# Wikinaut/agrep

Measured on NVIDIA H100. Metric: text_scan_throughput, higher is better.
Workload: dtype u32 bitwise

## Files before the change

### agrep_b200/csrc/refine.cu

```cuda
#include "scan_internal.cuh"


#define REFINE_MAXG  8
int refine_launch_u32a(int nrows, const RefineParams &P, unsigned &grid, cudaStream_t st);
int refine_launch_u32b(int nrows, const RefineParams &P, unsigned &grid, cudaStream_t st);
int refine_launch_u64(int nrows, const RefineParams &P, unsigned &grid, cudaStream_t st);
int refine_launch_costs(bool narrow, int nrows, const RefineParams &P, unsigned &grid, cudaStream_t st);

__global__ void __launch_bounds__(REFINE_THREADS)
k_compact_ranges(const uint32_t *bitmap, uint64_t n_words, const uint64_t *range_offsets, uint64_t *list, uint64_t cap)
{
	const uint32_t lane = threadIdx.x & 31;
	const uint64_t warp = ((uint64_t)blockIdx.x * REFINE_THREADS + threadIdx.x) >> 5, nwarps = ((uint64_t)gridDim.x * REFINE_THREADS) >> 5;
	const uint64_t n_groups = (n_words + 31) / 32, per = (n_groups + nwarps - 1) / nwarps;
	const uint64_t g_begin = warp * per < n_groups ? warp * per : n_groups, g_end = (g_begin + per < n_groups) ? g_begin + per : n_groups;
	uint64_t at = range_offsets[warp];
	for (uint64_t g0 = g_begin; g0 < g_end; g0 += 8) {
		uint32_t wd[8];
#pragma unroll
		for (int u = 0; u < 8; u++) { const uint64_t w = (g0 + u) * 32 + lane; wd[u] = (g0 + u < g_end && w < n_words) ? bitmap[w] : 0u; }
#pragma unroll
		for (int u = 0; u < 8; u++) {
			const uint32_t word = wd[u];
			if (!__ballot_sync(0xffffffffu, word != 0)) continue;
			const uint64_t w = (g0 + u) * 32 + lane;
			uint32_t c = __popc(word), pre = c;
#pragma unroll
			for (int o = 1; o < 32; o <<= 1) { uint32_t v = __shfl_up_sync(0xffffffffu, pre, o); if (lane >= (uint32_t)o) pre += v; }
			const uint32_t total = __shfl_sync(0xffffffffu, pre, 31);
			uint64_t mine = at + (pre - c);
			for (uint32_t b = word; b; b &= b - 1) { if (mine < cap) list[mine] = w * 32 + (uint64_t)(__ffs(b) - 1); mine++; }
			at += total;
		}
	}
}

static bool refine_geometry(const agb_desc &d, RefineParams &P)
{
	if (!front_usable(d) || !d.refine) return false;
	int max_off = 0, min_off = 1 << 30;
	for (int i = 0; i < d.n_anchors; i++) { max_off = std::max(max_off, (int)d.anchor_off[i]); min_off = std::min(min_off, (int)d.anchor_off[i]); }
	for (int i = 0; i < d.n_anchors3; i++) { max_off = std::max(max_off, (int)d.anchor3_off[i]); min_off = std::min(min_off, (int)d.anchor3_off[i]); }
	P.lo_off = max_off + d.k;
	P.hi_off = 15 + d.pat_len - min_off + d.k;
	P.gb = (P.lo_off + 15) / 16;
	P.ng = P.gb + (P.hi_off + 15) / 16;
	if (P.ng < P.gb + 2) P.ng = P.gb + 2;
	const int pw = (d.pat_len + 3) / 4, ngc = (d.engine != AGB_ENGINE_ASEARCH1 && d.M <= 31 && pw <= 4) ? 4 : REFINE_MAXG;
	if (!(P.ng <= ngc && max_off <= 31 && d.pat_len >= 1 && d.pat_len <= 64)) return false;
	const int na = d.n_anchors + d.n_anchors3;
	if (na > 16) return false;
	uint32_t val[16], msk[16]; int off[16];
	for (int i = 0; i < d.n_anchors; i++) { val[i] = d.anchor[i]; msk[i] = d.anchor_mask; off[i] = d.anchor_off[i]; }
	for (int i = 0; i < d.n_anchors3; i++) { val[d.n_anchors + i] = d.anchor3[i]; msk[d.n_anchors + i] = 0x00FFFFFFu; off[d.n_anchors + i] = d.anchor3_off[i]; }
	for (int i = 0; i < na; i++) for (int j = 0; j < i; j++) if ((val[i] & msk[j]) == val[j] || (val[j] & msk[i]) == val[i]) return false;
	uint32_t mul = 0x9E3779B1u;
	for (int attempt = 0; attempt < 4096; attempt++, mul = mul * 0x2C1B3C6Du + 0x297A2D39u) {
		int8_t slot[32]; bool ok = true;
		memset(slot, 0, sizeof slot);
		mul |= 1u;
		for (int i = 0; i < na && ok; i++) {
			const uint32_t h = (val[i] * mul) >> 27;
			if (slot[h]) ok = false; else slot[h] = (int8_t)(i + 1);
		}
		if (!ok) continue;
		P.hmul = mul;
		memcpy(P.hidx64, slot, sizeof slot);
		int8_t offs8[16];
		for (int i = 0; i < 16; i++) { P.hval[i] = i < na ? val[i] : 0; P.hmask[i] = i < na ? msk[i] : 0; offs8[i] = i < na ? (int8_t)off[i] : 0; }
		memcpy(P.hoffs64, offs8, sizeof offs8);
		return true;
	}
	return false;
}

static void refine_t1_setup(const agb_desc &d, RefineParams &P)
{
	uint8_t lit[64]; bool is_lit[64]; bool fold = false; int n_lit = 0;
	for (int j = 0; j < d.pat_len; j++) {
		const uint64_t bit = 1ull << (d.M - (d.L + 2 + j));
		int cnt = 0, c0 = -1, c1 = -1;
		for (int c = 0; c < 256; c++) if (d.mask[c] & bit) { if (cnt == 0) c0 = c; else if (cnt == 1) c1 = c; cnt++; }
		is_lit[j] = false; lit[j] = 0;
		if (cnt == 1 && c0 < 0x80) { is_lit[j] = true; lit[j] = (uint8_t)c0; }
		else if (cnt == 2 && (c0 ^ c1) == 0x20 && c1 < 0x80) { is_lit[j] = true; lit[j] = (uint8_t)(c0 | 0x20); fold = true; }
		if (is_lit[j]) n_lit++;
	}
	P.t1 = 0;
	if (n_lit <= d.k + 1) return;
	P.t1 = 1; P.t1_fold = fold ? 0x20202020u : 0u;
	for (int w = 0; w < 16; w++) { P.t1_pat[w] = 0; P.t1_care[w] = 0; }
	for (int j = 0; j < d.pat_len; j++) if (is_lit[j]) {
		P.t1_pat[j >> 2] |= (uint32_t)(fold ? (lit[j] | 0x20) : lit[j]) << (8 * (j & 3));
		P.t1_care[j >> 2] |= 0x80u << (8 * (j & 3));
	}
}

int refine_launch(const agb_desc &d, Workspace &W, const void *d_text, uint64_t n, cudaStream_t st, bool *ran)
{
	RefineParams P; memset(&P, 0, sizeof P);
	*ran = false;
	if (n == 0 || !refine_geometry(d, P)) return AGB_OK;
	const uint64_t n_chunks = (n + 15) / 16, n_words = (n_chunks + 31) / 32;
	P.text = (const uint8_t *)d_text; P.bitmap = W.bitmap; P.out = W.bitmap2; P.warp_counts = W.range_counts;
	P.n = n; P.n_chunks = n_chunks; P.n_words = n_words; P.desc = W.d_desc;
	P.fold = d.anchor_fold; P.amask = d.anchor_mask; P.na = d.n_anchors; P.k = d.k; P.pat_len = d.pat_len;
	for (int i = 0; i < d.n_anchors; i++) { P.anchor[i] = d.anchor[i]; P.off[i] = d.anchor_off[i]; }
	{
		bool distinct = true;
		for (int i = 0; i < d.n_anchors; i++) for (int j = 0; j < i; j++) if (d.anchor[i] == d.anchor[j]) distinct = false;
		P.one = 1; P.scale = 1;
		for (int i = d.anchor_len; i < 4; i++) P.scale <<= 8;
		P.poly = (distinct && poly_setup(d.anchor, d.n_anchors, 8 * d.anchor_len, P.coef)) ? 1 : 0;
		P.n3 = 0;
		if (d.n_anchors3) {
			uint32_t c3[AGB_MAXANCHOR];
			if (!P.poly || !poly_setup(d.anchor3, d.n_anchors3, 24, c3)) return AGB_OK;
			P.n3 = d.n_anchors3;
			for (int i = 0; i < d.n_anchors3; i++) P.coef3[i] = c3[i];
		}
	}
	refine_t1_setup(d, P);
	unsigned grid = refine_grid(W, n);
	P.sm_count = W.sm_count;
	const bool costs = d.engine == AGB_ENGINE_ASEARCH1, narrow = d.M <= 31;
	int rc = costs ? refine_launch_costs(narrow, d.nrows, P, grid, st)
	       : !narrow ? refine_launch_u64(d.nrows, P, grid, st)
	       : d.nrows <= 4 ? refine_launch_u32a(d.nrows, P, grid, st) : refine_launch_u32b(d.nrows, P, grid, st);
	if (rc) return AGB_ERR_ARG;
	g_launches++;
	CUDA_TRY(cudaGetLastError());
	W.refine_ctas = grid;
	*ran = true;
	return AGB_OK;
}

unsigned refine_grid(const Workspace &W, uint64_t n)
{
	const uint64_t n_chunks = (n + 15) / 16, n_words = (n_chunks + 31) / 32, groups = (n_words + 31) / 32;
	unsigned grid = (unsigned)std::min<uint64_t>((groups + 3) / 4, (uint64_t)W.sm_count * 16);
	return grid ? grid : 1;
}

int compact_ranges_launch(Workspace &W, uint64_t n, cudaStream_t st)
{
	const uint64_t n_chunks = (n + 15) / 16, n_words = (n_chunks + 31) / 32;
	const unsigned grid = W.refine_ctas;
	k_compact_ranges<<<grid, REFINE_THREADS, 0, st>>>(W.bitmap2, n_words, W.range_offsets, W.cand, W.cand_cap); g_launches++;
	CUDA_TRY(cudaGetLastError());
	return AGB_OK;
}
```

### agrep_b200/csrc/refine_kernel.cuh

```cuda
#ifndef AGB_REFINE_KERNEL_CUH
#define AGB_REFINE_KERNEL_CUH
#include "automaton.cuh"

#define REFINE_RING1 544
#define REFINE_RING2 64
#define REFINE_RING3 128
#define REFINE_MAXG  8
#define REFINE_PAD   32

struct AnchorTable { int8_t idx[32]; uint32_t val[16], mask[16]; int8_t off[16]; int n; };
__device__ __forceinline__ uint32_t hit_windows_tab(const uint32_t (&x)[5], const AnchorTable &A)
{
	uint32_t hits = 0;
#pragma unroll
	for (int w = 0; w < 4; w++) {
		const uint32_t wv[4] = { x[w], __funnelshift_r(x[w], x[w + 1], 8), __funnelshift_r(x[w], x[w + 1], 16), __funnelshift_r(x[w], x[w + 1], 24) };
		for (int a = 0; a < A.n; a++) {
			const uint32_t V = A.val[a], M = A.mask[a];
#pragma unroll
			for (int j = 0; j < 4; j++) if ((wv[j] & M) == V) hits |= 1u << (4 * w + j);
		}
	}
	return hits;
}

template <int NA, bool SCALED>
__device__ __forceinline__ uint32_t hit_windows_poly(const uint32_t (&x)[5], const RefineParams &P)
{
	uint32_t wv[16];
#pragma unroll
	for (int w = 0; w < 4; w++) {
		wv[4 * w] = x[w]; wv[4 * w + 1] = __funnelshift_r(x[w], x[w + 1], 8);
		wv[4 * w + 2] = __funnelshift_r(x[w], x[w + 1], 16); wv[4 * w + 3] = __funnelshift_r(x[w], x[w + 1], 24);
	}
	uint32_t nz = 0;
#pragma unroll
	for (int s = 15; s >= 0; s--) {
		uint32_t r = wv[s] * P.one + P.coef[NA - 1];
#pragma unroll
		for (int i = NA - 2; i >= 0; i--) r = r * wv[s] + P.coef[i];
		if (SCALED) r *= P.scale;
		nz = nz * 2u + min(r, 1u);
	}
	return ~nz & 0xFFFFu;
}
__device__ __forceinline__ uint32_t hit_windows_cmp(const uint32_t (&x)[5], const RefineParams &P)
{
	uint32_t hits = 0;
#pragma unroll
	for (int w = 0; w < 4; w++) {
		const uint32_t wv[4] = { x[w], __funnelshift_r(x[w], x[w + 1], 8), __funnelshift_r(x[w], x[w + 1], 16), __funnelshift_r(x[w], x[w + 1], 24) };
		for (int a = 0; a < P.na; a++) {
			const uint32_t A = P.anchor[a];
#pragma unroll
			for (int j = 0; j < 4; j++) if ((wv[j] & P.amask) == A) hits |= 1u << (4 * w + j);
		}
	}
	return hits;
}
template <bool SCALED>
__device__ __forceinline__ uint32_t hit_windows_na(const uint32_t (&x)[5], const RefineParams &P)
{
	switch (P.na) {
	case 1: return hit_windows_poly<1, SCALED>(x, P);  case 2: return hit_windows_poly<2, SCALED>(x, P);
	case 3: return hit_windows_poly<3, SCALED>(x, P);  case 4: return hit_windows_poly<4, SCALED>(x, P);
	case 5: return hit_windows_poly<5, SCALED>(x, P);  case 6: return hit_windows_poly<6, SCALED>(x, P);
	case 7: return hit_windows_poly<7, SCALED>(x, P);  case 8: return hit_windows_poly<8, SCALED>(x, P);
	default: return hit_windows_poly<9, SCALED>(x, P);
	}
}
__device__ __forceinline__ uint32_t hit_windows(const uint32_t (&x)[5], const RefineParams &P)
{
	if (!P.poly) return hit_windows_cmp(x, P);
	return P.scale != 1 ? hit_windows_na<true>(x, P) : hit_windows_na<false>(x, P);
}

__device__ __forceinline__ uint32_t start_code(const uint32_t *cw, const int s, const RefineParams &P, const AnchorTable &A)
{
	const uint32_t lo = cw[s >> 2] | P.fold, hi = cw[(s >> 2) + 1] | P.fold;
	const uint32_t v = __funnelshift_r(lo, hi, (s & 3) * 8);
	int off = 0;
	{
		const uint32_t v4 = v & P.amask;
		const int i = A.idx[(v4 * P.hmul) >> 27];
		if (i && A.val[i - 1] == (v & A.mask[i - 1])) off = A.off[i - 1];
		else if (P.n3) {
			const uint32_t v3 = v & 0x00FFFFFFu;
			const int i3 = A.idx[(v3 * P.hmul) >> 27];
			if (i3 && A.val[i3 - 1] == (v & A.mask[i3 - 1])) off = A.off[i3 - 1];
		}
	}
	return (uint32_t)(32 + s - off);
}

template <int NW, int NWT, int ND>
__device__ __forceinline__ bool band_count_passes(const RefineParams &P, const uint32_t *strip, const int so)
{
	uint32_t W[NWT + 1];
	{
		const uint32_t *src = strip + (so >> 2);
		const uint32_t sh = ((uint32_t)so & 3u) * 8u;
		uint32_t Lw[NWT + 1];
#pragma unroll
		for (int i = 0; i <= NWT; i++) Lw[i] = src[i];
#pragma unroll
		for (int i = 0; i < NWT; i++) W[i] = (__funnelshift_r(Lw[i], Lw[i + 1], sh) & 0x7F7F7F7Fu) | P.t1_fold;
		W[NWT] = 0;
	}
	uint32_t acc[NW];
#pragma unroll
	for (int w = 0; w < NW; w++) acc[w] = 0x80808080u;
	const int nd = ND ? ND : 2 * P.k + 1;
#pragma unroll (ND ? ND : 1)
	for (int d = 0; d < nd; d++) {
#pragma unroll
		for (int w = 0; w < NW; w++) acc[w] &= (W[w] ^ P.t1_pat[w]) + 0x7F7F7F7Fu;
#pragma unroll
		for (int i = 0; i < NWT; i++) W[i] = __funnelshift_r(W[i], W[i + 1], 8);
	}
	int miss = 0;
#pragma unroll
	for (int w = 0; w < NW; w++) miss += __popc(acc[w] & P.t1_care[w]);
	return miss <= P.k;
}

template <typename T, int NR, bool COSTS>
__device__ __forceinline__ bool window_passes(const uint8_t *bytes, const bool run, const int wlen, const T init0,
                                              const T *mask, const DevConsts<T> &C)
{
	T S[NR];
#pragma unroll
	for (int r = 0; r < NR; r++) S[r] = init0;
	int q = 0;
	for (; q + 4 <= wlen; q += 4) {
		int c[4];
#pragma unroll
		for (int i = 0; i < 4; i++) c[i] = run ? (int)__ldg(bytes + q + i) : 0;
		T m[4];
#pragma unroll
		for (int i = 0; i < 4; i++) m[i] = mask[c[i]];
#pragma unroll
		for (int i = 0; i < 4; i++) rows_step<T, NR, COSTS>(S, m[i], C);
	}
	for (; q < wlen; q++) {
		const int c = run ? (int)__ldg(bytes + q) : 0;
		rows_step<T, NR, COSTS>(S, mask[c], C);
	}
	return run && (S[NR - 1] & C.endpos) != 0;
}

struct Refill { uint32_t word, next_word; uint32_t half; };
__device__ __forceinline__ void refine_refill(const RefineParams &P, Refill &R, uint32_t *ring, uint32_t &count, uint32_t lane,
                                              uint64_t &g, uint64_t g_begin, uint64_t g_end)
{
	if (R.half == 0) {
		const uint64_t w = g * 32 + lane;
		R.word = R.next_word;
		if (w < P.n_words) P.out[w] = 0u;
		R.next_word = (g + 1 < g_end && w + 32 < P.n_words) ? P.bitmap[w + 32] : 0u;
	}
	const uint32_t word = ((lane >> 4) == R.half) ? R.word : 0u;
	uint32_t c = __popc(word), pre = c;
#pragma unroll
	for (int o = 1; o < 32; o <<= 1) { uint32_t v = __shfl_up_sync(0xffffffffu, pre, o); if (lane >= (uint32_t)o) pre += v; }
	const uint32_t total = __shfl_sync(0xffffffffu, pre, 31);
	pre += count - c;
	const uint32_t rel0 = (uint32_t)(g - g_begin) * 1024u + lane * 32u;
	for (uint32_t b = word; b; b &= b - 1) ring[pre++] = rel0 + (uint32_t)(__ffs(b) - 1);
	count += total;
	if (R.half) g++;
	R.half ^= 1u;
	__syncwarp();
}

template <typename T, int NR, bool COSTS, int NW>
__global__ void __launch_bounds__(REFINE_THREADS, 6)
k_refine(const RefineParams P)
{
	constexpr int NGC = NW <= 4 ? 4 : REFINE_MAXG;
	constexpr int NWT = NW + (2 * (NR - 1) + 3) / 4;
	extern __shared__ __align__(16) uint32_t s_strip[];
	__shared__ RecShared<T, NR> SH;
	__shared__ uint32_t s_ring1[REFINE_THREADS / 32][REFINE_RING1];
	__shared__ uint32_t s_ring2[REFINE_THREADS / 32][REFINE_RING2];
	__shared__ uint32_t s_ring3[REFINE_THREADS / 32][REFINE_RING3];
	__shared__ AnchorTable s_offs;
	if (threadIdx.x == 0) {
#pragma unroll
		for (int i = 0; i < 32; i++) s_offs.idx[i] = (int8_t)(P.hidx64[i >> 3] >> (8 * (i & 7)));
#pragma unroll
		s_offs.n = P.na + P.n3;
#pragma unroll
		for (int i = 0; i < 16; i++) { s_offs.val[i] = P.hval[i]; s_offs.mask[i] = P.hmask[i]; s_offs.off[i] = (int8_t)(P.hoffs64[i >> 3] >> (8 * (i & 7))); }
	}
	DevConsts<T> C;
	shared_init<T, NR>(SH, C, P.desc, REFINE_THREADS);
	const T init0 = mirror<T>((T)P.desc->init0);
	const int wlen = P.pat_len + 2 * P.k;
	const uint32_t lane = threadIdx.x & 31, wib = threadIdx.x >> 5, lt_mask = (1u << lane) - 1u;
	uint32_t *ring1 = s_ring1[wib], *ring2 = s_ring2[wib], *ring3 = s_ring3[wib];
	const int stride_w = P.ng * 4 + 1;
	uint32_t *strip = s_strip + threadIdx.x * stride_w;
	const uint32_t *cw = strip + P.gb * 4;
	const int so0 = P.gb * 16 - 32 - P.k;

	const uint64_t warp = ((uint64_t)blockIdx.x * REFINE_THREADS + threadIdx.x) >> 5, nwarps = ((uint64_t)gridDim.x * REFINE_THREADS) >> 5;
	const uint64_t n_groups = (P.n_words + 31) / 32, per = (n_groups + nwarps - 1) / nwarps;
	const uint64_t g_begin = warp * per < n_groups ? warp * per : n_groups, g_end = (g_begin + per < n_groups) ? g_begin + per : n_groups;
	const uint64_t chunk0 = g_begin * 1024;
	uint32_t rel_lo, rel_hi;
	{
		const int64_t lo_chunk = ((int64_t)P.lo_off + 15) / 16;
		int64_t hi_chunk = ((int64_t)P.n - P.hi_off - 16) / 16;
		if ((int64_t)P.n - P.hi_off - 16 < 0) hi_chunk = -1;
		if (hi_chunk > (int64_t)P.n_chunks - 3) hi_chunk = (int64_t)P.n_chunks - 3;
		const int64_t a = lo_chunk - (int64_t)chunk0, b = hi_chunk - (int64_t)chunk0;
		rel_lo = a < 0 ? 0u : (a > 0x7fffffff ? 0x7fffffffu : (uint32_t)a);
		rel_hi = b < 0 ? 0u : (b > 0x7fffffff ? 0x7fffffffu : (uint32_t)b);
		if (b < 0) rel_lo = 0x7fffffffu;
	}
	const uint4 *text4 = reinterpret_cast<const uint4 *>(P.text) + chunk0;
	uint32_t kept = 0;
	auto keep_chunk = [&](uint32_t rel) {
		const uint64_t chunk = chunk0 + rel;
		const uint32_t bit = 1u << (chunk & 31);
		const uint32_t old = atomicOr(&P.out[chunk >> 5], bit);
		kept += (old & bit) ? 0u : 1u;
	};

	uint32_t n1 = 0, n2 = 0, n3 = 0;
	uint64_t g = g_begin;
	Refill RF; RF.word = 0; RF.half = 0;
	RF.next_word = (g < g_end && g * 32 + lane < P.n_words) ? P.bitmap[g * 32 + lane] : 0u;
	auto fill1 = [&]() { while (n1 < 32 && g < g_end) refine_refill(P, RF, ring1, n1, lane, g, g_begin, g_end); };
	uint32_t nrel = 0; bool nrun = false, nedge = false; uint4 nx[NGC];
	auto pop_load = [&](uint32_t rel, bool active) {
		nrel = rel;
		nedge = active && (rel < rel_lo || rel > rel_hi);
		nrun = active && !nedge;
		if (nrun) {
			const uint4 *src = text4 + ((int64_t)rel - P.gb);
#pragma unroll
			for (int gi = 0; gi < NGC; gi++) if (gi < P.ng) nx[gi] = __ldg(src + gi);
		}
	};
	auto to_strip = [&]() {
#pragma unroll
		for (int gi = 0; gi < NGC; gi++) if (gi < P.ng) {
			strip[gi * 4 + 0] = nx[gi].x; strip[gi * 4 + 1] = nx[gi].y; strip[gi * 4 + 2] = nx[gi].z; strip[gi * 4 + 3] = nx[gi].w;
		}
	};
	auto count_push = [&](uint32_t rel, uint32_t code, bool run) {
		const bool pass = run && (!P.t1 || band_count_passes<NW, NWT, COSTS ? 0 : 2 * (NR - 1) + 1>(P, strip, so0 + (int)code));
		const uint32_t pm = __ballot_sync(0xffffffffu, pass);
		if (pass) ring3[n3 + __popc(pm & lt_mask)] = (rel << 6) | code;
		n3 += __popc(pm);
	};
	auto walk_batch = [&]() {
		const uint32_t m = n3 < 32 ? n3 : 32;
		const bool run = lane < m;
		const uint32_t e = run ? ring3[n3 - m + lane] : 0u;
		n3 -= m;
		const uint8_t *wbytes = P.text + ((int64_t)(chunk0 + (e >> 6)) * 16 + (int64_t)(e & 63u) - 32 - P.k);
		if (window_passes<T, NR, COSTS>(run ? wbytes : P.text, run, wlen, init0, SH.mask, C)) keep_chunk(e >> 6);
		__syncwarp();
	};
	auto more_batch = [&]() {
		const uint32_t m = n2 < 32 ? n2 : 32;
		const bool run = lane < m;
		const uint32_t e = run ? ring2[n2 - m + lane] : 0u;
		n2 -= m;
		const uint32_t rel = e >> 6, first = e & 63u;
		if (run) {
			const uint4 *src = text4 + ((int64_t)rel - P.gb);
#pragma unroll
			for (int gi = 0; gi < NGC; gi++) if (gi < P.ng) {
				const uint4 v = __ldg(src + gi);
				strip[gi * 4 + 0] = v.x; strip[gi * 4 + 1] = v.y; strip[gi * 4 + 2] = v.z; strip[gi * 4 + 3] = v.w;
			}
		}
		uint32_t hits = 0;
		if (run) {
			const uint32_t x[5] = { cw[0] | P.fold, cw[1] | P.fold, cw[2] | P.fold, cw[3] | P.fold, cw[4] | P.fold };
			hits = P.n3 ? hit_windows_tab(x, s_offs) : hit_windows(x, P);
			hits &= hits - 1;
		}
		uint32_t seen1 = first, seen2 = first;
		for (int it = 0; it < 3; it++) {
			if (!__ballot_sync(0xffffffffu, hits != 0)) break;
			uint32_t code = first; bool fresh = false;
			if (hits) {
				code = start_code(cw, __ffs(hits) - 1, P, s_offs);
				hits &= hits - 1;
				fresh = code != first && code != seen1 && code != seen2;
				seen2 = seen1; seen1 = code;
			}
			count_push(rel, code, fresh);
		}
		if (hits) keep_chunk(rel);
		__syncwarp();
	};
	auto pop1 = [&]() {
		const uint32_t m = n1 < 32 ? n1 : 32;
		const bool active = lane < m;
		pop_load(active ? ring1[n1 - m + lane] : 0u, active);
		n1 -= m;
	};

	bool have = false;
	for (;;) {
		if (n3 >= 32) { walk_batch(); continue; }
		if (n2 >= 32) { more_batch(); continue; }
		if (!have) {
			fill1();
			if (n1 == 0) break;
			pop1(); have = true;
			continue;
		}
		const uint32_t crel = nrel; const bool crun = nrun, cedge = nedge;
		if (crun) to_strip();
		fill1();
		have = n1 != 0;
		if (have) pop1();
		if (cedge) keep_chunk(crel);
		uint32_t hits = 0, code = 0;
		if (crun) {
			const uint32_t x[5] = { cw[0] | P.fold, cw[1] | P.fold, cw[2] | P.fold, cw[3] | P.fold, cw[4] | P.fold };
			hits = P.n3 ? hit_windows_tab(x, s_offs) : hit_windows(x, P);
			if (hits) code = start_code(cw, __ffs(hits) - 1, P, s_offs);
		}
		count_push(crel, code, hits != 0);
		{
			uint32_t rest = hits & (hits - 1);
			if (rest && !(rest & (rest - 1)) && start_code(cw, __ffs(rest) - 1, P, s_offs) == code) rest = 0;
			const bool more = rest != 0;
			const uint32_t mm = __ballot_sync(0xffffffffu, more);
			if (more) ring2[n2 + __popc(mm & lt_mask)] = (crel << 6) | code;
			n2 += __popc(mm);
		}
		__syncwarp();
	}
	while (n2 || n3) { if (n3 >= 32 || !n2) walk_batch(); else more_batch(); }
	const uint32_t total = __reduce_add_sync(0xffffffffu, kept);
	if (lane == 0) P.warp_counts[warp] = total;
}

template <typename T, int NR, bool COSTS, int NW>
static void launch_refine_nw(const RefineParams &P, unsigned &grid, cudaStream_t st)
{
	const size_t smem = ((size_t)REFINE_THREADS * (P.ng * 4 + 1) + REFINE_PAD) * sizeof(uint32_t);
	int per_sm = 0;
	if (cudaOccupancyMaxActiveBlocksPerMultiprocessor(&per_sm, k_refine<T, NR, COSTS, NW>, REFINE_THREADS, smem) != cudaSuccess || per_sm < 1) per_sm = 4;
	grid = std::min<unsigned>(grid, (unsigned)per_sm * (unsigned)P.sm_count);
	if (!grid) grid = 1;
	k_refine<T, NR, COSTS, NW><<<grid, REFINE_THREADS, smem, st>>>(P);
}
template <typename T, int NR, bool COSTS>
static void launch_refine_one(const RefineParams &P, unsigned &grid, cudaStream_t st)
{
	const int pw = (P.pat_len + 3) / 4;
	if (COSTS) { if (sizeof(T) == 4) launch_refine_nw<T, NR, COSTS, 8>(P, grid, st); else launch_refine_nw<T, NR, COSTS, 16>(P, grid, st); return; }
	if (sizeof(T) == 4) {
		if (pw <= 2) launch_refine_nw<T, NR, COSTS, 2>(P, grid, st);
		else if (pw == 3) launch_refine_nw<T, NR, COSTS, 3>(P, grid, st);
		else if (pw == 4) launch_refine_nw<T, NR, COSTS, 4>(P, grid, st);
		else if (pw <= 6) launch_refine_nw<T, NR, COSTS, 6>(P, grid, st);
		else launch_refine_nw<T, NR, COSTS, 8>(P, grid, st);
	} else {
		if (pw <= 8) launch_refine_nw<T, NR, COSTS, 8>(P, grid, st);
		else if (pw <= 12) launch_refine_nw<T, NR, COSTS, 12>(P, grid, st);
		else launch_refine_nw<T, NR, COSTS, 16>(P, grid, st);
	}
}

#endif
```

### agrep_b200/csrc/scan_internal.cuh

```cuda
#ifndef AGB_SCAN_INTERNAL_CUH
#define AGB_SCAN_INTERNAL_CUH
#include "agrep_b200.h"
#include "pattern_internal.h"
#include <cuda_runtime.h>
#include <stdint.h>
#include <stdio.h>
#include <string.h>
#include <stdlib.h>
#include <atomic>
#include <algorithm>

extern thread_local char g_err[512];
extern std::atomic<uint64_t> g_launches;

#define CUDA_TRY(x) do { cudaError_t e_ = (x); if (e_ != cudaSuccess) { \
	snprintf(g_err, sizeof g_err, "%s failed: %s (%s:%d)", #x, cudaGetErrorString(e_), __FILE__, __LINE__); \
	return AGB_ERR_CUDA; } } while (0)

#define FRONT_THREADS 256
#define FRONT_CH      4
#define FRONT_STAGE_CHUNKS (FRONT_THREADS * FRONT_CH)
#define FRONT_STAGE_BYTES  (FRONT_STAGE_CHUNKS * 16)
#define FRONT_SLOT_BYTES   (FRONT_STAGE_BYTES + 16)
#define FRONT_NST     2
#define FRONT_CTAS_PER_SM 6
#define FRONT_WORDS_PER_STAGE (FRONT_STAGE_CHUNKS / 32)

struct FrontParams {
	const uint8_t *text;
	uint32_t    *bitmap;
	uint64_t     n;
	uint64_t     n_chunks;
	uint64_t     readable;
	uint64_t     stage_begin, stage_end;
	uint32_t     fold, amask;
	uint32_t     one, scale;
	uint32_t     anchor[AGB_MAXANCHOR];
	uint32_t     coef[AGB_MAXANCHOR];
	int          n3;
	uint32_t     s256;
	int          alen;
	uint32_t     coef3[4];
	uint16_t    *nl_blocks;
	uint32_t     delim4, dfold4;
};
#define FRONT_SMEM (FRONT_NST * FRONT_SLOT_BYTES)

#define REFINE_THREADS 128
struct RefineParams {
	const uint8_t *text; const uint32_t *bitmap; uint32_t *out; uint32_t *warp_counts;
	uint64_t n, n_chunks, n_words;
	const agb_desc *desc;
	uint32_t fold, amask; int na, k, pat_len;
	int gb, ng;
	int lo_off, hi_off;
	uint32_t anchor[AGB_MAXANCHOR]; int32_t off[AGB_MAXANCHOR];
	uint32_t coef[AGB_MAXANCHOR]; uint32_t one, scale; int poly;
	int t1, t1_words;
	uint32_t t1_fold, t1_pat[16], t1_care[16];
	uint32_t hmul; uint64_t hidx64[4];
	uint32_t hval[16], hmask[16]; uint64_t hoffs64[2];
	int n3; uint32_t coef3[4];
	int sm_count;
};

#define REC_THREADS 128

struct RecParams {
	const uint8_t  *text;
	uint64_t n, n_chunks;
	const agb_desc *desc;
	uint32_t *tile_counts;
	const uint64_t *tile_offsets;
	agb_record *records; uint64_t capacity;
	unsigned long long *totals;
	const uint64_t *cand; uint64_t cand_cap;
	agb_record *cand_first;
	int emit;
	int levels;
	int want_level;
	int warm;
	int64_t own_lo, own_hi; int shard_last;
	const void *rx_tab; int rx_tail;
	const struct SetFile *set_files; const struct SetTile *set_tiles; unsigned long long *set_stats;
};
struct SetFile { uint64_t off, n; uint32_t ord_tile0; int32_t j0; };
struct SetTile { uint32_t file, tile; };
#define SET_STATS 16
struct ShardInfo { int64_t own_lo, own_hi; int last; };
#define DENSE_THREADS 256
#define DENSE_TILE    32768
#define RX_TILE       32768
#define DENSE_TAIL    2048
#define DENSE_PER     (DENSE_TILE / DENSE_THREADS)
#define DENSE_SMEM (DENSE_TILE + DENSE_TAIL)
#define SL_THREADS 128
#define SL_PER     256
#define SL_TILE    (SL_THREADS * SL_PER)
#define SL_APRON   128
#define SL_STRIDE  (SL_PER + 4)
#define SL_SMEM    ((SL_THREADS + 1) * SL_STRIDE + 12)
#define COMPACT_THREADS 256
#define COMPACT_WPT 4
#define SCAN_BLOCK 16384
static inline bool list_form_pays(uint64_t flagged, uint64_t n_chunks) { return flagged <= n_chunks / 20 + 1024; }

#define ORD_THREADS 256
#define ORD_TILE    32768
#define ORD_PER     (ORD_TILE / ORD_THREADS)
#define ORD_BLOCK   512

struct OrdParams {
	const uint8_t *text; uint64_t n;
	uint16_t *blocks; uint32_t *tiles; const uint64_t *tile_off;
	agb_record *records; const unsigned long long *totals; uint64_t capacity;
	uint8_t delim[AGB_MAXDELIM + 2], dfold[AGB_MAXDELIM + 2]; int L, kind;
	long long j0;
};

__device__ __forceinline__ bool rec_owned(const RecParams &P, int64_t begin, int L, int64_t close_pos)
{
	const int64_t oe = begin + L - 1;
	if (oe < P.own_lo || oe >= P.own_hi) return false;
	if (!P.shard_last && close_pos >= (int64_t)P.n) P.totals[11] = 1ull;
	return true;
}

#define H2D_SLICE   (64ull << 20)
#define STAGE_BUFS  3
struct Workspace {
	uint32_t *bitmap = nullptr; size_t bitmap_bytes = 0;
	uint32_t *bitmap2 = nullptr;
	uint32_t *range_counts = nullptr; uint64_t *range_offsets = nullptr;
	unsigned refine_ctas = 0;
	uint32_t *d_gram = nullptr; unsigned int *h_gram = nullptr;
	uint64_t plan_key = 0; bool plan_valid = false; agb_desc plan_desc;
	size_t cand_hint = 0;
	uint32_t *tile_counts = nullptr; uint64_t *tile_offsets = nullptr; size_t tiles = 0;
	uint64_t *cand = nullptr; uint32_t *cand_counts = nullptr; uint64_t *cand_offsets = nullptr; agb_record *cand_first = nullptr; size_t cand_cap = 0;
	uint32_t *scan_sums = nullptr; uint64_t *scan_offs = nullptr; size_t scan_cap = 0;
	uint16_t *ord_blocks = nullptr; size_t ord_blocks_cap = 0;
	long long ord_j0 = 0;
	int ord_virt = 0;
	unsigned long long *totals = nullptr;
	unsigned long long *h_totals = nullptr;
	agb_desc *d_desc = nullptr; agb_desc h_desc_copy; bool desc_valid = false;
	cudaEvent_t e0 = nullptr, e1 = nullptr, e2 = nullptr;
	int sm_count = 0;
	uint64_t *d_regex = nullptr; uint64_t h_regex[8 * 256]; size_t regex_bytes = 0; int regex_tail = 0;
};

#include <mutex>
extern Workspace g_ws[64];
extern std::mutex g_ws_mu[64];
int  scan_device_impl(const agb_desc &d, const void *d_text, uint64_t n, int want, int want_level,
                      agb_record *d_records, uint64_t capacity, cudaStream_t st, agb_result *res, const ShardInfo *sh = nullptr,
                      const agb_pattern *px = nullptr);
enum { HALO_SHORT_RIGHT = 1, HALO_SHORT_LEFT = 2 };
int  shard_window_scan(const agb_desc &d, const agb_pattern *px, const void *d_win, uint64_t n_local, uint64_t halo_left, uint64_t halo_right,
                       bool first, bool open_end, bool reaches_end, int want, agb_record *d_records, uint64_t capacity,
                       cudaStream_t st, agb_result *lres, agb_shard_part *part);
int  shard_window_rebase(agb_record *d_records, uint64_t n, long long byte_add, long long ord_add, bool ordinals, cudaStream_t st);
bool front_usable(const agb_desc &d);
bool exact_count_usable(const agb_desc &d);
int  exact_count_launch(const agb_desc &d, Workspace &W, const void *d_text, uint64_t n, cudaStream_t st);
bool poly_setup(const uint32_t *a, int na, int bits, uint32_t *coef);
int  front_launch(const agb_desc &d, Workspace &W, const void *d_text, uint64_t n, uint64_t word_begin, uint64_t word_end, bool slack16, cudaStream_t st, bool count_delims = false);
int  refine_launch(const agb_desc &d, Workspace &W, const void *d_text, uint64_t n, cudaStream_t st, bool *ran);
unsigned refine_grid(const Workspace &W, uint64_t n);
int  compact_ranges_launch(Workspace &W, uint64_t n, cudaStream_t st);
#define REFINE_MAX_RANGES 16384
int  launch_dense(const agb_desc &d, const RecParams &P, unsigned grid, cudaStream_t st);
int  launch_dense_set(const agb_desc &d, const RecParams &P, unsigned grid, cudaStream_t st);
int  launch_regex_set(const agb_desc &d, const RecParams &P, unsigned grid, cudaStream_t st);
int  launch_records_list(const agb_desc &d, const RecParams &P, unsigned grid, cudaStream_t st);
int  launch_dense_wide(int nrows, const RecParams &P, unsigned grid, cudaStream_t st, bool set);
int  launch_records_list_wide(int nrows, const RecParams &P, unsigned grid, cudaStream_t st);
int  launch_slices(const agb_desc &d, const RecParams &P, unsigned grid, cudaStream_t st);
bool slices_usable(const agb_desc &d);
int  launch_regex(const agb_desc &d, const RecParams &P, unsigned grid, cudaStream_t st);
size_t regex_tables(const agb_desc &d, const agb_regex &rx, uint64_t *out);
__global__ void k_gram_sample(const uint8_t *text, uint64_t n_chunks, uint32_t nblk, uint32_t blk_chunks,
                              int ngram, const uint32_t *gram, const uint32_t *gmask, uint32_t fold, unsigned int *counts,
                              int pair_first, int n_pair);
__global__ void k_compact_count(const uint32_t *bitmap, uint64_t n_words, uint32_t *block_counts, unsigned long long *totals);
__global__ void k_compact_write(const uint32_t *bitmap, uint64_t n_words, const uint64_t *block_offsets, uint64_t *cand, uint64_t cand_cap);
__global__ void k_scan_tiles(const uint32_t *counts, uint64_t *offsets, uint64_t n_tiles, unsigned long long *total);
__global__ void k_scan_partial(const uint32_t *counts, uint64_t n, uint32_t *block_sums, const unsigned long long *n_dev);
__global__ void k_scan_apply(const uint32_t *counts, uint64_t n, const uint64_t *block_offsets, uint64_t *offsets, const unsigned long long *n_dev);
int  front_is_dense(Workspace &W, uint64_t n, cudaStream_t st, bool *dense);
int  ordinals_launch(const agb_desc &d, Workspace &W, const void *d_text, uint64_t n, agb_record *d_records, uint64_t capacity, cudaStream_t st, bool blocks_counted = false);
int  ordinals_reserve(const agb_desc &d, Workspace &W, uint64_t n);
int  ordinals_set_launch(const agb_desc &d, Workspace &W, const void *d_text, const SetFile *d_files, const SetTile *d_ord_tiles,
                         uint64_t ord_tiles, unsigned long long *d_stats, agb_record *d_records, uint64_t capacity, cudaStream_t st);
__device__ __forceinline__ void set_enter(const SetFile *files, const SetTile *tiles, const uint8_t *&text, uint64_t &n,
                                          uint64_t &tile, uint32_t &file)
{
	const SetTile t = tiles[blockIdx.x];
	const SetFile f = files[t.file];
	text += f.off; n = f.n; tile = t.tile; file = t.file;
}
#endif
```

Measured before the change: 2308.

## Replace polynomial/hash anchor matching with per-anchor start bitmasks in refine

Drops the polynomial-root anchor test, the hashed anchor table and the secondary ring2 'more starts' queue. Each anchor is now tested with a single scaled multiply-add per window, and the hits are packed into a 64-bit mask of candidate start codes that is drained one code per loop iteration through count_push. This removes the hash lookups, the shared AnchorTable and the extra batching pass, in exchange for na separate passes over the 16 windows and possibly more loop iterations per chunk. Patterns with up to 9 anchors are accepted instead of 16.

Measured after the change: 2328 (median of 6 runs). Within noise of the previous version (+0.9%).

```diff
diff --git a/agrep_b200/csrc/refine.cu b/agrep_b200/csrc/refine.cu
--- a/agrep_b200/csrc/refine.cu
+++ b/agrep_b200/csrc/refine.cu
@@ -49,29 +49,19 @@
 	const int pw = (d.pat_len + 3) / 4, ngc = (d.engine != AGB_ENGINE_ASEARCH1 && d.M <= 31 && pw <= 4) ? 4 : REFINE_MAXG;
 	if (!(P.ng <= ngc && max_off <= 31 && d.pat_len >= 1 && d.pat_len <= 64)) return false;
 	const int na = d.n_anchors + d.n_anchors3;
-	if (na > 16) return false;
-	uint32_t val[16], msk[16]; int off[16];
-	for (int i = 0; i < d.n_anchors; i++) { val[i] = d.anchor[i]; msk[i] = d.anchor_mask; off[i] = d.anchor_off[i]; }
-	for (int i = 0; i < d.n_anchors3; i++) { val[d.n_anchors + i] = d.anchor3[i]; msk[d.n_anchors + i] = 0x00FFFFFFu; off[d.n_anchors + i] = d.anchor3_off[i]; }
+	if (na > REFINE_MAXA) return false;
+	uint32_t val[REFINE_MAXA], msk[REFINE_MAXA];
+	for (int i = 0; i < d.n_anchors; i++) { val[i] = d.anchor[i]; msk[i] = d.anchor_mask; }
+	for (int i = 0; i < d.n_anchors3; i++) { val[d.n_anchors + i] = d.anchor3[i]; msk[d.n_anchors + i] = 0x00FFFFFFu; }
 	for (int i = 0; i < na; i++) for (int j = 0; j < i; j++) if ((val[i] & msk[j]) == val[j] || (val[j] & msk[i]) == val[i]) return false;
-	uint32_t mul = 0x9E3779B1u;
-	for (int attempt = 0; attempt < 4096; attempt++, mul = mul * 0x2C1B3C6Du + 0x297A2D39u) {
-		int8_t slot[32]; bool ok = true;
-		memset(slot, 0, sizeof slot);
-		mul |= 1u;
-		for (int i = 0; i < na && ok; i++) {
-			const uint32_t h = (val[i] * mul) >> 27;
-			if (slot[h]) ok = false; else slot[h] = (int8_t)(i + 1);
-		}
-		if (!ok) continue;
-		P.hmul = mul;
-		memcpy(P.hidx64, slot, sizeof slot);
-		int8_t offs8[16];
-		for (int i = 0; i < 16; i++) { P.hval[i] = i < na ? val[i] : 0; P.hmask[i] = i < na ? msk[i] : 0; offs8[i] = i < na ? (int8_t)off[i] : 0; }
-		memcpy(P.hoffs64, offs8, sizeof offs8);
-		return true;
+	P.na = na;
+	for (int i = 0; i < na; i++) {
+		const bool three = i >= d.n_anchors;
+		P.ascale[i] = three ? 256u : 1u << (8 * (4 - d.anchor_len));
+		P.acoef[i] = 0u - val[i] * P.ascale[i];
+		P.ashift[i] = 32 - (three ? d.anchor3_off[i - d.n_anchors] : d.anchor_off[i]);
 	}
-	return false;
+	return true;
 }
 
 static void refine_t1_setup(const agb_desc &d, RefineParams &P)
@@ -104,22 +94,7 @@
 	const uint64_t n_chunks = (n + 15) / 16, n_words = (n_chunks + 31) / 32;
 	P.text = (const uint8_t *)d_text; P.bitmap = W.bitmap; P.out = W.bitmap2; P.warp_counts = W.range_counts;
 	P.n = n; P.n_chunks = n_chunks; P.n_words = n_words; P.desc = W.d_desc;
-	P.fold = d.anchor_fold; P.amask = d.anchor_mask; P.na = d.n_anchors; P.k = d.k; P.pat_len = d.pat_len;
-	for (int i = 0; i < d.n_anchors; i++) { P.anchor[i] = d.anchor[i]; P.off[i] = d.anchor_off[i]; }
-	{
-		bool distinct = true;
-		for (int i = 0; i < d.n_anchors; i++) for (int j = 0; j < i; j++) if (d.anchor[i] == d.anchor[j]) distinct = false;
-		P.one = 1; P.scale = 1;
-		for (int i = d.anchor_len; i < 4; i++) P.scale <<= 8;
-		P.poly = (distinct && poly_setup(d.anchor, d.n_anchors, 8 * d.anchor_len, P.coef)) ? 1 : 0;
-		P.n3 = 0;
-		if (d.n_anchors3) {
-			uint32_t c3[AGB_MAXANCHOR];
-			if (!P.poly || !poly_setup(d.anchor3, d.n_anchors3, 24, c3)) return AGB_OK;
-			P.n3 = d.n_anchors3;
-			for (int i = 0; i < d.n_anchors3; i++) P.coef3[i] = c3[i];
-		}
-	}
+	P.fold = d.anchor_fold; P.k = d.k; P.pat_len = d.pat_len;
 	refine_t1_setup(d, P);
 	unsigned grid = refine_grid(W, n);
 	P.sm_count = W.sm_count;
diff --git a/agrep_b200/csrc/refine_kernel.cuh b/agrep_b200/csrc/refine_kernel.cuh
--- a/agrep_b200/csrc/refine_kernel.cuh
+++ b/agrep_b200/csrc/refine_kernel.cuh
@@ -3,29 +3,11 @@
 #include "automaton.cuh"
 
 #define REFINE_RING1 544
-#define REFINE_RING2 64
-#define REFINE_RING3 128
+#define REFINE_RING3 64
 #define REFINE_MAXG  8
 #define REFINE_PAD   32
 
-struct AnchorTable { int8_t idx[32]; uint32_t val[16], mask[16]; int8_t off[16]; int n; };
-__device__ __forceinline__ uint32_t hit_windows_tab(const uint32_t (&x)[5], const AnchorTable &A)
-{
-	uint32_t hits = 0;
-#pragma unroll
-	for (int w = 0; w < 4; w++) {
-		const uint32_t wv[4] = { x[w], __funnelshift_r(x[w], x[w + 1], 8), __funnelshift_r(x[w], x[w + 1], 16), __funnelshift_r(x[w], x[w + 1], 24) };
-		for (int a = 0; a < A.n; a++) {
-			const uint32_t V = A.val[a], M = A.mask[a];
-#pragma unroll
-			for (int j = 0; j < 4; j++) if ((wv[j] & M) == V) hits |= 1u << (4 * w + j);
-		}
-	}
-	return hits;
-}
-
-template <int NA, bool SCALED>
-__device__ __forceinline__ uint32_t hit_windows_poly(const uint32_t (&x)[5], const RefineParams &P)
+__device__ __forceinline__ uint64_t chunk_starts(const uint32_t (&x)[5], const RefineParams &P)
 {
 	uint32_t wv[16];
 #pragma unroll
@@ -33,64 +15,16 @@
 		wv[4 * w] = x[w]; wv[4 * w + 1] = __funnelshift_r(x[w], x[w + 1], 8);
 		wv[4 * w + 2] = __funnelshift_r(x[w], x[w + 1], 16); wv[4 * w + 3] = __funnelshift_r(x[w], x[w + 1], 24);
 	}
-	uint32_t nz = 0;
-#pragma unroll
-	for (int s = 15; s >= 0; s--) {
-		uint32_t r = wv[s] * P.one + P.coef[NA - 1];
-#pragma unroll
-		for (int i = NA - 2; i >= 0; i--) r = r * wv[s] + P.coef[i];
-		if (SCALED) r *= P.scale;
-		nz = nz * 2u + min(r, 1u);
-	}
-	return ~nz & 0xFFFFu;
-}
-__device__ __forceinline__ uint32_t hit_windows_cmp(const uint32_t (&x)[5], const RefineParams &P)
-{
-	uint32_t hits = 0;
-#pragma unroll
-	for (int w = 0; w < 4; w++) {
-		const uint32_t wv[4] = { x[w], __funnelshift_r(x[w], x[w + 1], 8), __funnelshift_r(x[w], x[w + 1], 16), __funnelshift_r(x[w], x[w + 1], 24) };
-		for (int a = 0; a < P.na; a++) {
-			const uint32_t A = P.anchor[a];
-#pragma unroll
-			for (int j = 0; j < 4; j++) if ((wv[j] & P.amask) == A) hits |= 1u << (4 * w + j);
-		}
-	}
-	return hits;
-}
-template <bool SCALED>
-__device__ __forceinline__ uint32_t hit_windows_na(const uint32_t (&x)[5], const RefineParams &P)
-{
-	switch (P.na) {
-	case 1: return hit_windows_poly<1, SCALED>(x, P);  case 2: return hit_windows_poly<2, SCALED>(x, P);
-	case 3: return hit_windows_poly<3, SCALED>(x, P);  case 4: return hit_windows_poly<4, SCALED>(x, P);
-	case 5: return hit_windows_poly<5, SCALED>(x, P);  case 6: return hit_windows_poly<6, SCALED>(x, P);
-	case 7: return hit_windows_poly<7, SCALED>(x, P);  case 8: return hit_windows_poly<8, SCALED>(x, P);
-	default: return hit_windows_poly<9, SCALED>(x, P);
-	}
-}
-__device__ __forceinline__ uint32_t hit_windows(const uint32_t (&x)[5], const RefineParams &P)
-{
-	if (!P.poly) return hit_windows_cmp(x, P);
-	return P.scale != 1 ? hit_windows_na<true>(x, P) : hit_windows_na<false>(x, P);
-}
-
-__device__ __forceinline__ uint32_t start_code(const uint32_t *cw, const int s, const RefineParams &P, const AnchorTable &A)
-{
-	const uint32_t lo = cw[s >> 2] | P.fold, hi = cw[(s >> 2) + 1] | P.fold;
-	const uint32_t v = __funnelshift_r(lo, hi, (s & 3) * 8);
-	int off = 0;
-	{
-		const uint32_t v4 = v & P.amask;
-		const int i = A.idx[(v4 * P.hmul) >> 27];
-		if (i && A.val[i - 1] == (v & A.mask[i - 1])) off = A.off[i - 1];
-		else if (P.n3) {
-			const uint32_t v3 = v & 0x00FFFFFFu;
-			const int i3 = A.idx[(v3 * P.hmul) >> 27];
-			if (i3 && A.val[i3 - 1] == (v & A.mask[i3 - 1])) off = A.off[i3 - 1];
-		}
-	}
-	return (uint32_t)(32 + s - off);
+	uint64_t starts = 0;
+#pragma unroll
+	for (int i = 0; i < REFINE_MAXA; i++) {
+		if (i >= P.na) break;
+		uint32_t nz = 0;
+#pragma unroll
+		for (int s = 15; s >= 0; s--) nz = nz * 2u + min(wv[s] * P.ascale[i] + P.acoef[i], 1u);
+		starts |= (uint64_t)(~nz & 0xFFFFu) << P.ashift[i];
+	}
+	return starts;
 }
 
 template <int NW, int NWT, int ND>
@@ -182,23 +116,13 @@
 	extern __shared__ __align__(16) uint32_t s_strip[];
 	__shared__ RecShared<T, NR> SH;
 	__shared__ uint32_t s_ring1[REFINE_THREADS / 32][REFINE_RING1];
-	__shared__ uint32_t s_ring2[REFINE_THREADS / 32][REFINE_RING2];
 	__shared__ uint32_t s_ring3[REFINE_THREADS / 32][REFINE_RING3];
-	__shared__ AnchorTable s_offs;
-	if (threadIdx.x == 0) {
-#pragma unroll
-		for (int i = 0; i < 32; i++) s_offs.idx[i] = (int8_t)(P.hidx64[i >> 3] >> (8 * (i & 7)));
-#pragma unroll
-		s_offs.n = P.na + P.n3;
-#pragma unroll
-		for (int i = 0; i < 16; i++) { s_offs.val[i] = P.hval[i]; s_offs.mask[i] = P.hmask[i]; s_offs.off[i] = (int8_t)(P.hoffs64[i >> 3] >> (8 * (i & 7))); }
-	}
 	DevConsts<T> C;
 	shared_init<T, NR>(SH, C, P.desc, REFINE_THREADS);
 	const T init0 = mirror<T>((T)P.desc->init0);
 	const int wlen = P.pat_len + 2 * P.k;
 	const uint32_t lane = threadIdx.x & 31, wib = threadIdx.x >> 5, lt_mask = (1u << lane) - 1u;
-	uint32_t *ring1 = s_ring1[wib], *ring2 = s_ring2[wib], *ring3 = s_ring3[wib];
+	uint32_t *ring1 = s_ring1[wib], *ring3 = s_ring3[wib];
 	const int stride_w = P.ng * 4 + 1;
 	uint32_t *strip = s_strip + threadIdx.x * stride_w;
 	const uint32_t *cw = strip + P.gb * 4;
@@ -228,7 +152,7 @@
 		kept += (old & bit) ? 0u : 1u;
 	};
 
-	uint32_t n1 = 0, n2 = 0, n3 = 0;
+	uint32_t n1 = 0, n3 = 0;
 	uint64_t g = g_begin;
 	Refill RF; RF.word = 0; RF.half = 0;
 	RF.next_word = (g < g_end && g * 32 + lane < P.n_words) ? P.bitmap[g * 32 + lane] : 0u;
@@ -265,41 +189,6 @@
 		if (window_passes<T, NR, COSTS>(run ? wbytes : P.text, run, wlen, init0, SH.mask, C)) keep_chunk(e >> 6);
 		__syncwarp();
 	};
-	auto more_batch = [&]() {
-		const uint32_t m = n2 < 32 ? n2 : 32;
-		const bool run = lane < m;
-		const uint32_t e = run ? ring2[n2 - m + lane] : 0u;
-		n2 -= m;
-		const uint32_t rel = e >> 6, first = e & 63u;
-		if (run) {
-			const uint4 *src = text4 + ((int64_t)rel - P.gb);
-#pragma unroll
-			for (int gi = 0; gi < NGC; gi++) if (gi < P.ng) {
-				const uint4 v = __ldg(src + gi);
-				strip[gi * 4 + 0] = v.x; strip[gi * 4 + 1] = v.y; strip[gi * 4 + 2] = v.z; strip[gi * 4 + 3] = v.w;
-			}
-		}
-		uint32_t hits = 0;
-		if (run) {
-			const uint32_t x[5] = { cw[0] | P.fold, cw[1] | P.fold, cw[2] | P.fold, cw[3] | P.fold, cw[4] | P.fold };
-			hits = P.n3 ? hit_windows_tab(x, s_offs) : hit_windows(x, P);
-			hits &= hits - 1;
-		}
-		uint32_t seen1 = first, seen2 = first;
-		for (int it = 0; it < 3; it++) {
-			if (!__ballot_sync(0xffffffffu, hits != 0)) break;
-			uint32_t code = first; bool fresh = false;
-			if (hits) {
-				code = start_code(cw, __ffs(hits) - 1, P, s_offs);
-				hits &= hits - 1;
-				fresh = code != first && code != seen1 && code != seen2;
-				seen2 = seen1; seen1 = code;
-			}
-			count_push(rel, code, fresh);
-		}
-		if (hits) keep_chunk(rel);
-		__syncwarp();
-	};
 	auto pop1 = [&]() {
 		const uint32_t m = n1 < 32 ? n1 : 32;
 		const bool active = lane < m;
@@ -308,39 +197,36 @@
 	};
 
 	bool have = false;
+	uint32_t crel = 0; uint64_t starts = 0;
 	for (;;) {
 		if (n3 >= 32) { walk_batch(); continue; }
-		if (n2 >= 32) { more_batch(); continue; }
+		if (__any_sync(0xffffffffu, starts != 0)) {
+			const bool run = starts != 0;
+			const uint32_t code = run ? (uint32_t)(__ffsll((long long)starts) - 1) : 0u;
+			starts &= starts - 1;
+			count_push(crel, code, run);
+			continue;
+		}
 		if (!have) {
 			fill1();
 			if (n1 == 0) break;
 			pop1(); have = true;
 			continue;
 		}
-		const uint32_t crel = nrel; const bool crun = nrun, cedge = nedge;
+		crel = nrel;
+		const bool crun = nrun, cedge = nedge;
 		if (crun) to_strip();
 		fill1();
 		have = n1 != 0;
 		if (have) pop1();
 		if (cedge) keep_chunk(crel);
-		uint32_t hits = 0, code = 0;
 		if (crun) {
 			const uint32_t x[5] = { cw[0] | P.fold, cw[1] | P.fold, cw[2] | P.fold, cw[3] | P.fold, cw[4] | P.fold };
-			hits = P.n3 ? hit_windows_tab(x, s_offs) : hit_windows(x, P);
-			if (hits) code = start_code(cw, __ffs(hits) - 1, P, s_offs);
-		}
-		count_push(crel, code, hits != 0);
-		{
-			uint32_t rest = hits & (hits - 1);
-			if (rest && !(rest & (rest - 1)) && start_code(cw, __ffs(rest) - 1, P, s_offs) == code) rest = 0;
-			const bool more = rest != 0;
-			const uint32_t mm = __ballot_sync(0xffffffffu, more);
-			if (more) ring2[n2 + __popc(mm & lt_mask)] = (crel << 6) | code;
-			n2 += __popc(mm);
+			starts = chunk_starts(x, P);
 		}
 		__syncwarp();
 	}
-	while (n2 || n3) { if (n3 >= 32 || !n2) walk_batch(); else more_batch(); }
+	while (n3) walk_batch();
 	const uint32_t total = __reduce_add_sync(0xffffffffu, kept);
 	if (lane == 0) P.warp_counts[warp] = total;
 }
@@ -359,8 +245,8 @@
 static void launch_refine_one(const RefineParams &P, unsigned &grid, cudaStream_t st)
 {
 	const int pw = (P.pat_len + 3) / 4;
-	if (COSTS) { if (sizeof(T) == 4) launch_refine_nw<T, NR, COSTS, 8>(P, grid, st); else launch_refine_nw<T, NR, COSTS, 16>(P, grid, st); return; }
-	if (sizeof(T) == 4) {
+	if constexpr (COSTS) { if constexpr (sizeof(T) == 4) launch_refine_nw<T, NR, COSTS, 8>(P, grid, st); else launch_refine_nw<T, NR, COSTS, 16>(P, grid, st); return; }
+	else if constexpr (sizeof(T) == 4) {
 		if (pw <= 2) launch_refine_nw<T, NR, COSTS, 2>(P, grid, st);
 		else if (pw == 3) launch_refine_nw<T, NR, COSTS, 3>(P, grid, st);
 		else if (pw == 4) launch_refine_nw<T, NR, COSTS, 4>(P, grid, st);
diff --git a/agrep_b200/csrc/scan_internal.cuh b/agrep_b200/csrc/scan_internal.cuh
--- a/agrep_b200/csrc/scan_internal.cuh
+++ b/agrep_b200/csrc/scan_internal.cuh
@@ -47,20 +47,17 @@
 #define FRONT_SMEM (FRONT_NST * FRONT_SLOT_BYTES)
 
 #define REFINE_THREADS 128
+#define REFINE_MAXA    9
 struct RefineParams {
 	const uint8_t *text; const uint32_t *bitmap; uint32_t *out; uint32_t *warp_counts;
 	uint64_t n, n_chunks, n_words;
 	const agb_desc *desc;
-	uint32_t fold, amask; int na, k, pat_len;
+	uint32_t fold; int na, k, pat_len;
 	int gb, ng;
 	int lo_off, hi_off;
-	uint32_t anchor[AGB_MAXANCHOR]; int32_t off[AGB_MAXANCHOR];
-	uint32_t coef[AGB_MAXANCHOR]; uint32_t one, scale; int poly;
+	uint32_t ascale[REFINE_MAXA], acoef[REFINE_MAXA]; int32_t ashift[REFINE_MAXA];
 	int t1, t1_words;
 	uint32_t t1_fold, t1_pat[16], t1_care[16];
-	uint32_t hmul; uint64_t hidx64[4];
-	uint32_t hval[16], hmask[16]; uint64_t hoffs64[2];
-	int n3; uint32_t coef3[4];
 	int sm_count;
 };
 
```
